# ninalu/urlearning-cpp

Measured on AMD Instinct MI355X. Metric: cBIC parent-set scores/sec + A* expansions/sec, n=25 full skeleton, higher is better.
Workload: dtype f64; 1 GPU; C3 cBIC scoring: n=25, N=10000, max-parents k=6, lambda=2.0, full n x n skeleton, 25 variables balanced over 1 GPU(s), one all-gather of the lists; config_id=c3, mode=shard, parallelism=variable shard x1, steps_in_flight=3

## Files before the change

urlearning-cpp_amd/csrc/cbic.hip:

```cpp
#include <cstdio>
#include <atomic>
#include <thread>
#include <algorithm>
#include <chrono>
#include <cmath>
#include <cstdlib>
#include <cstring>

#include "search_internal.h"
#include "host_walk.h"
#include "cbic_dev.h"

using namespace ulg;

namespace {

typedef double f64x4 __attribute__((ext_vector_type(4)));

constexpr int kGramRows = 1024;


__device__ double block_sum(double v, double *red) {
    red[threadIdx.x] = v;
    __syncthreads();
// ... 82 lines not shown


struct ScoreArgs {
    const double *gram;
    const uint32_t *binom;
    const uint8_t *cand;
    const int *meta;
    const uint64_t *tbl_off;
    const uint64_t *work;
    uint64_t total;
    float *table;
    float *hsub;
    uint64_t *queue;
    unsigned long long *qcount;
    unsigned long long *err;
    uint8_t *qkey;
    double N;
    double pen;
    int n, nv, S;
    int xcd;
    int hsub_out;
    const uint32_t *lut;
    const int32_t *lut_off;
};

__device__ __forceinline__ uint32_t xcd_block(uint32_t b, uint32_t nb, int on) {
    if (!on) return b;
    const uint32_t x = b & 7u, k = b >> 3, q = nb >> 3, r = nb & 7u;
    return x * q + (x < r ? x : r) + k;
}

__host__ __device__ inline bool cons_violates(const uint64_t *ct, int nv, int vi, uint64_t set) {
    const uint64_t b = ct[vi], e = ct[vi + 1];
    if (b == e) return false;
    const uint64_t *p = ct + nv + 1 + 2 * b;
    for (uint64_t i = 0; i < e - b; ++i)
        if ((p[2 * i] & ~set) == 0 && (p[2 * i + 1] & set) == 0) return false;
    return true;
}
template <int THREADS>
__device__ __forceinline__ const uint64_t *cons_stage(unsigned char *smem, int lds_end, const uint64_t *cons,
                                                      int cons_words) {
    if (cons_words > kConsLdsWords) return cons;
    uint64_t *sc = reinterpret_cast<uint64_t *>(smem + ((lds_end + 15) & ~15));
    for (int i = threadIdx.x; i < cons_words; i += THREADS) sc[i] = cons[i];
    return sc;
}


struct LdsLayout {
    int gram, binom, work, lutoff, toff, meta, cand, stack, bits, cmp, cmp2, total;
};
constexpr int kCmpEntryBytes = 8 + 4 + 4 + 4 + 4;
__host__ __device__ inline int align16(int x) { return (x + 15) & ~15; }
#ifndef ULG_LDS_ALIAS
#define ULG_LDS_ALIAS 1
#endif
__host__ __device__ inline LdsLayout lds_layout(int n, int nv, int S, int L, int V) {
    LdsLayout l;
    if (ULG_LDS_ALIAS && (V & 208) == 208 && bits_words(L) < 4) {
        const int W = bits_words(L);
        l.binom = 0;
        l.toff = align16(l.binom + 64 * kBinomK * 4);
        l.meta = align16(l.toff + (nv * S + 1) * 8);
        l.cmp = align16(l.meta + nv * 4 * 4);
        const int ra = l.cmp + 16;
        l.gram = ra;
        l.work = align16(l.gram + n * n * 8);
        l.lutoff = l.work + (nv + 1) * 8;
        l.cand = align16(l.lutoff + nv * 4);
        l.stack = l.bits = align16(l.cand + nv * 64);
        l.cmp2 = align16(ra + kBlock * kCmpEntryBytes);
        const int endc = l.cmp2 + 2 * W * kBlock * 8;
        l.total = l.stack > endc ? l.stack : endc;
        return l;
    }
    l.gram = 0;
    l.binom = align16(l.gram + n * n * 8);
    l.work = align16(l.binom + 64 * kBinomK * 4);
    l.lutoff = l.work + (nv + 1) * 8;
    l.toff = align16(l.lutoff + nv * 4);
    l.meta = align16(l.toff + (nv * S + 1) * 8);
    l.cand = align16(l.meta + nv * 4 * 4);
    l.stack = align16(l.cand + nv * 64);
    l.bits = l.stack;
    const int W = bits_words(L);
    l.cmp = align16(l.bits + (W >= 4 ? 3 * W * kBlock * 8 : 0));
    l.cmp2 = align16(l.cmp + ((V & 80) == 80 ? 16 + kBlock * kCmpEntryBytes : 0));
    l.total = l.cmp2 + ((V & 208) == 208 && W < 4 ? 2 * W * kBlock * 8 : 0);
    return l;
}



constexpr unsigned long long kErrWide = 1ull, kErrQueue = 2ull, kErrSlot = 4ull;
__device__ __forceinline__ uint64_t walk_segment() { return blockIdx.x % seg_count(gridDim.x); }

template <int L, int PHASE, int W>
__device__ __forceinline__ uint32_t walk_key(const uint64_t (&ow)[W]) {
    constexpr uint32_t root = PHASE == 0 ? ((1u << L) - 1u) : (((1u << L) - 1u) << 1);
    constexpr int off = PHASE == 0 ? 0 : 1;
    uint32_t key = 0;
#pragma unroll
    for (int a = 0; a < L; ++a) {
        const uint32_t t = root ^ (1u << (a + off));
        key |= (uint32_t)((ow[t >> 6] >> (t & 63u)) & 1ull) << a;
    }
    if (key == (1u << L) - 1u) {
        uint32_t sec = 0;
        int nb = 0;
#pragma unroll
        for (int a = 0; a < L; ++a)
#pragma unroll
// ... 2085 lines not shown
        if (cnt == 0) continue;
        if ((cnt + kBlock - 1) / kBlock > 0x7fffffffull)
            return set_err(k.c, ULG_ERR_UNSUPPORTED, "ulg_cbic_score: layer too large");
        const size_t wo = p.work_offset(g, L, ph);
        wide.push_back(wide_group(k, g, L, ph, k.d_wk + wo, p.group_work().data() + wo, cnt));
    }
    return wide.empty() ? ULG_OK : score_wide_groups(k, L, ph, wide, k.c->wide_pinned);
}

int launch_prologue(const ScoreCall &k) {
    ulg_ctx *c = k.c;
    const CbicPlan &p = k.p;
    const uint64_t nqc = p.zero_q ? p.nqc : 0;
    const uint64_t nz = std::max<uint64_t>((uint64_t)p.nv, std::max<uint64_t>(nqc, p.nqseg));
    const dim3 grid((unsigned)((nz + 255) / 256)), block(256);
    unsigned long long *qcount = p.zero_q ? c->d_qcount.p : nullptr, *qseg = p.zero_q ? c->d_qseg.p : nullptr;
    if (k.cons.words)
        return launch_kernel(c, call_prologue_cons_kernel, grid, block, 0, c->stream, "call_prologue", c->d_tbl_off.p,
                             p.nv, k.ls.S, c->table.p, qcount, nqc, qseg, p.nqseg, k.cons.dev, k.ls.n);
    return launch_kernel(c, call_prologue_kernel, grid, block, 0, c->stream, "call_prologue", c->d_tbl_off.p, p.nv,
                         k.ls.S, c->table.p, qcount, nqc, qseg, p.nqseg);
}

int launch_small(const ScoreCall &k, int L, int ph) {
    ulg_ctx *c = k.c;
    const CbicPlan &p = k.p;
    const int n = k.ls.n, nv = p.nv, S = k.ls.S;
    ScoreArgs ss = k.sa;
    if (L <= p.Lf) {
        if (L != 1 || ph != 0) return ULG_OK;
        ss.hsub_out = p.Lf < p.kmax;
        return launch_twin(c, k.cons, small_kernel<false>(p.Lf), small_kernel<true>(p.Lf), dim3((unsigned)nv),
                           dim3(kFusedThreads), lds_layout(n, nv, S, p.Lf, 65).total, c->stream, "score_small_fused",
                           ss, (const uint64_t *)c->d_work.p);
    }
    const size_t wo = p.work_offset(0, L, ph);
    const uint64_t cnt = p.work[wo + nv];
    if (cnt == 0) return ULG_OK;
    ss.work = c->d_work.p + wo;
    ss.total = cnt;
    ss.lut_off = p.lut_any ? c->d_lutoff.p + p.lut_offset(L, ph) : nullptr;
    ss.hsub_out = !(L == p.kmax && ph == 1);
    return launch_twin(c, k.cons, layer_kernel<false>(L, ph, p.vsmall), layer_kernel<true>(L, ph, p.vsmall),
                       dim3((unsigned)((cnt + kBlock - 1) / kBlock)), dim3(kBlock),
                       lds_layout(n, nv, S, L, p.vsmall).total, c->stream, kLayerNames[ph][L], ss);
}

int walk_bucketed(const ScoreCall &k, int g, int L, int ph, const ScoreArgs &sa, uint64_t blocks, int wk) {
    ulg_ctx *c = k.c;
    const CbicPlan &p = k.p;
    hipStream_t st = k.gst[g];
    const unsigned long long *qc = sa.qcount;
    const uint64_t nseg = seg_count(blocks);
    const int kl = L == 6 ? (wk >= 8 ? 8 : 4) : (wk >= 4 ? 4 : 2);
    uint32_t *kbase = c->d_qoffs.p + (size_t)g * kBucketMax * p.nseg_max;
    uint32_t *sidx = c->d_qsidx.p + (size_t)g * p.qcap;
    uint32_t *qaux = c->d_qaux.p + (size_t)g * p.qcap;
    const unsigned int *hdr = reinterpret_cast<const unsigned int *>(qc + nseg * kSegStride);
    prof_begin_s(c, kWalkNames[ph][L], st);
    walk_bucket_count_kernel<<<(unsigned)((nseg + kBucketSegs - 1) / kBucketSegs), 256, 0, st>>>(
        qc, (uint32_t)nseg, L, sa.qkey, qaux, kbase);
    const uint64_t items = nseg * (kSegEntries / 256);
    walk_bucket_scatter_kernel<<<(unsigned)std::min<uint64_t>(items, 2048), 256, 0, st>>>(qc, qaux, kbase,
                                                                                          (uint32_t)nseg, L, sidx);
// ... 19 lines not shown
                       sa.hsub_out ? sa.hsub : nullptr, wck ? c->d_dump.p : nullptr, k.ls.total_slots, sa.err);
    prof_end_s(c, st);
    if (wck && (rc = dump_walk_clock(c, st, sb, wck, L, ph))) return rc;
    if (wck && std::getenv("ULG_WALK_QUEUE_DUMP") &&
        (rc = dump_walk_queue(c, st, sa.queue, sa.qcount, seg_count(blocks), bits_words(L), k.ls.total_slots, wck, L,
                              ph)))
        return rc;
    return ULG_OK;
}

int launch_unrolled(const ScoreCall &k, int g, int L, int ph) {
    ulg_ctx *c = k.c;
    const CbicPlan &p = k.p;
    const uint64_t cnt = p.launch_count(g, L, ph);
    if (cnt == 0) return ULG_OK;
    const uint64_t blocks = (cnt + kBlock - 1) / kBlock;
    if (blocks > 0x7fffffffull) return set_err(c, ULG_ERR_UNSUPPORTED, "ulg_cbic_score: layer too large");
    const bool two_pass = (p.variant & 16) != 0;
    const bool bk = p.bucket && (L == 5 || L == 6);
    ScoreArgs sa = k.sa;
    sa.work = k.d_wk + p.work_offset(g, L, ph);
    sa.total = cnt;
    sa.lut_off = p.lut_any ? c->d_lutoff.p + p.lut_offset(L, ph) : nullptr;
    sa.queue = two_pass ? c->d_queue.p + (size_t)g * p.qwords : nullptr;
    sa.qcount = two_pass ? c->d_qseg.p + p.segoff[p.seg_slot(g, L, ph)] : nullptr;
    sa.qkey = bk ? c->d_qkey.p + (size_t)g * p.qcap : nullptr;
    sa.hsub_out = !(L == p.kmax && ph == 1);
    int rc;
    if ((rc = launch_twin(c, k.cons, layer_kernel<false>(L, ph, p.variant), layer_kernel<true>(L, ph, p.variant),
                          dim3((unsigned)blocks), dim3(kBlock), lds_layout(k.ls.n, p.nv, k.ls.S, L, p.variant).total,
                          k.gst[g], kLayerNames[ph][L], sa)))
        return rc;
    if (!two_pass) return ULG_OK;
    const int wk = sliced_k(L, cnt, (uint64_t)c->walk_small_sets, c->walk_k6);
    if (bk) return walk_bucketed(k, g, L, ph, sa, blocks, wk);
    if ((p.variant & 32) && sliced_fn(L, ph, wk)) return walk_sliced(k, g, L, ph, sa, blocks, wk);
    return ULG_OK;
}

int launch_layers(const ScoreCall &k, int &done_L) {
    ulg_ctx *c = k.c;
    const CbicPlan &p = k.p;
    const int G = p.G, kmax = p.kmax;
    const auto t_call = std::chrono::steady_clock::now();
    int rc;
    bool forked = false;
// ... 73 lines not shown
        (rc = ensure(c, c->gram, (size_t)(n * n))) || (rc = ensure(c, c->colstat, (size_t)(2 * n))) ||
        (rc = ensure(c, c->partials, (size_t)chunks * tiles * tiles * 256)))
        return rc;
    ULG_HIP(c, hipMemcpyAsync(c->raw.p, data, sizeof(double) * (size_t)(N * n), hipMemcpyHostToDevice, c->stream));
    prof_begin(c, "colstats");
    colstats_kernel<<<n, kBlock, 0, c->stream>>>(c->raw.p, N, c->colstat.p);
    prof_end(c);
    const int64_t tot = N * c->npad;
    prof_begin(c, "normalise");
    normalise_kernel<<<(unsigned)((tot + kBlock - 1) / kBlock), kBlock, 0, c->stream>>>(c->raw.p, N, n, c->npad,
                                                                                         c->colstat.p, c->z.p);
    prof_end(c);
    prof_begin(c, "gram_mfma_f64");
    gram_mfma_kernel<<<dim3(chunks, tiles * tiles), 64, 0, c->stream>>>(c->z.p, N, c->npad, tiles, c->partials.p);
    prof_end(c);
    prof_begin(c, "gram_reduce");
    gram_reduce_kernel<<<(n * n + kBlock - 1) / kBlock, kBlock, 0, c->stream>>>(c->partials.p, chunks, tiles, n,
                                                                               c->gram.p);
    prof_end(c);
    if ((rc = ensure(c, c->d_pen, 1))) return rc;
    penalty_kernel<<<1, 1, 0, c->stream>>>((double)N, lambda, c->d_pen.p);
    ULG_HIP(c, hipGetLastError());
    ULG_HIP(c, hipMemcpyAsync(&c->pen, c->d_pen.p, sizeof(double), hipMemcpyDeviceToHost, c->stream));
    ULG_HIP(c, hipStreamSynchronize(c->stream));
    prof_collect(c);
    c->loaded = true;
    return ULG_OK;
}

int ulg_cbic_gram(ulg_ctx *c, double *out) {
    if (!c || !out) return ULG_ERR_ARG;
    if (!c->loaded) return set_err(c, ULG_ERR_STATE, "ulg_cbic_gram: no data loaded");
    ULG_HIP(c, hipSetDevice(c->device));
    ULG_HIP(c, hipMemcpy(out, c->gram.p, sizeof(double) * (size_t)(c->n * c->n), hipMemcpyDeviceToHost));
    return ULG_OK;
}

int ulg_cbic_score_finish(ulg_ctx *c, int64_t *total_stored, int64_t *total_scored) {
    if (!c) return ULG_ERR_ARG;
    if (c->async_pending) {
        c->async_pending = false;
        ULG_HIP(c, hipSetDevice(c->device));
        ULG_HIP(c, hipStreamSynchronize(c->stream));
        prof_collect(c);
        c->total_stored = (int64_t)c->async_pinned[0];
        c->last_err_word = c->async_pinned[1];
// ... 86 lines not shown
            if (c->wide_pinned) (void)hipHostFree(c->wide_pinned);
            c->wide_pinned = nullptr;
            ULG_HIP(c, hipHostMalloc((void **)&c->wide_pinned, sizeof(unsigned long long) * 2 * (size_t)G,
                                     hipHostMallocDefault));
            c->wide_host.assign(2 * G, 0);
        }
    }
    return ensure(c, c->d_blk, (size_t)p.nb + 2);
}

void graph_key(const ulg_ctx *c, const ScoreLists &ls, const CbicPlan &p, const uint64_t *candidates,
               std::vector<uint64_t> &gkey) {
    auto ptr = [](const void *q) { return (uint64_t)(uintptr_t)q; };
    gkey.assign({(uint64_t)ls.nv, (uint64_t)ls.max_parents, (uint64_t)p.variant, (uint64_t)p.G, (uint64_t)p.Ls,
                 (uint64_t)c->score_xcd, (uint64_t)ls.n, (uint64_t)c->N, dbits(c->lambda), (uint64_t)c->prof,
                 (uint64_t)c->walk_small_sets, (uint64_t)c->walk_k6, (uint64_t)c->walk_bucket, ptr(c->d_qaux.p),
                 ptr(c->d_qsidx.p), ptr(c->d_qkey.p), ptr(c->d_qoffs.p), ptr(c->table.p), ptr(c->d_work.p),
                 ptr(c->d_workg.p), ptr(c->d_queue.p), ptr(c->d_qcount.p), ptr(c->d_qseg.p), ptr(c->d_cand.p),
                 ptr(c->d_meta.p), ptr(c->d_tbl_off.p), ptr(c->out_sets.p), ptr(c->out_scores.p),
                 ptr(c->out_offsets.p), ptr(c->d_blk.p), ptr(c->gram.p), ptr(c->d_binom.p), ptr(c->d_binom64.p),
                 ptr(c->d_hsub.p), (uint64_t)ls.total_slots, (uint64_t)c->score_small_layers, (uint64_t)c->score_fused,
                 (uint64_t)p.cons_words, ptr(p.cons_words ? c->d_cons.p : nullptr), dbits(c->pen),
                 (uint64_t)c->score_unrank_lut, ptr(p.lut_any ? c->d_lut.p : nullptr),
                 ptr(p.lut_any ? c->d_lutoff.p : nullptr)});
    for (int i = 0; i < ls.nv; ++i) gkey.push_back((uint64_t)ls.vars[i]);
    for (int i = 0; i < ls.nv; ++i) gkey.push_back(candidates[i]);
    for (const std::string &nm : c->prof_only) gkey.push_back(std::hash<std::string>{}(nm));
}

int compact(const ScoreCall &k, int done_L) {
    ulg_ctx *c = k.c;
    const ScoreLists &ls = k.ls;
    const int nv = ls.nv, S = ls.S;
    const int64_t nb = k.p.nb;
    for (int i = 0; i < nv && done_L < ls.kmax; ++i) {
        const uint64_t b = ls.toff[(size_t)i * S + done_L + 1], e = ls.toff[(size_t)i * S + S];
        if (e > b) ULG_HIP(c, hipMemsetAsync(c->table.p + b, 0xff, (size_t)(e - b) * 4, c->stream));
    }
    c->completed_layer = done_L;
    prof_begin(c, "count_stored");
    count_kernel<<<(unsigned)nb, kBlock, 0, c->stream>>>(c->table.p, ls.total_slots, c->d_blk.p);
    prof_end(c);
    prof_begin(c, "scan_stored");
    scan_kernel<<<1, 1024, 0, c->stream>>>(c->d_blk.p, nb, c->out_offsets.p + nv, k.errf());
    prof_end(c);
    const WriteArgs wa{c->table.p,      c->d_blk.p,    c->d_tbl_off.p,  c->d_meta.p,      c->d_cand.p, c->d_binom.p,
                       c->d_binom64.p,  ls.total_slots, nv,             S,                c->out_sets.p,
// ... 76 lines not shown

int cbic_score(ulg_ctx *c, const int *vars, int nv, const uint64_t *candidates, int max_parents,
               int64_t *total_stored, int64_t *total_scored, bool async) {
    if (!c) return ULG_ERR_ARG;
    if (int rc0 = finish_pending(c)) return rc0;
    if (!c->loaded) return set_err(c, ULG_ERR_STATE, "ulg_cbic_score: call ulg_cbic_load first");
    ScoreLists &ls = c->lists;
    CbicPlan &p = c->plan;
    if (ScoreLists::Status st = ls.build(c->n, vars, nv, candidates, max_parents))
        return lists_error(c, "ulg_cbic_score", st);
    ULG_HIP(c, hipSetDevice(c->device));
    CbicOptions o;
    o.score_variant = c->score_variant;
    o.score_streams = c->score_streams;
    o.score_small_layers = c->score_small_layers;
    o.score_fused = c->score_fused;
    o.walk_bucket = c->walk_bucket;
    o.wide_prune = c->wide_prune;
    o.wide_pool = c->wide_pool;
    o.time_limit_ms = c->time_limit_ms;
    const char *wck = std::getenv("ULG_WALK_CLOCK");
    o.wck = wck != nullptr;
    o.score_unrank_lut = c->score_unrank_lut;
    p.build(ls, c->cons_var, c->cons_req, c->cons_forb, o);
    LutCache staged = c->lut_cache;
    p.build_luts(ls, o.score_unrank_lut, staged);
    if (int rc = reserve_buffers(c, ls, p)) return rc;
    if (int rc = reserve_luts(c, p, staged)) return rc;

    ScoreCall k{c, ls, p, ConsTable{p.cons_words ? c->d_cons.p : nullptr, p.cons_words, p.cons_lds}, ScoreArgs{},
                p.G > 1 ? c->d_workg.p : c->d_work.p, std::vector<hipStream_t>(p.G), wck};
    k.gst[0] = c->stream;
    for (int g = 1; g < p.G; ++g) k.gst[g] = c->aux_streams[g - 1];
    ScoreArgs &sa = k.sa;
    sa.hsub_out = 1;
    sa.gram = c->gram.p;
    sa.binom = c->d_binom.p;
    sa.cand = c->d_cand.p;
    sa.meta = c->d_meta.p;
    sa.tbl_off = c->d_tbl_off.p;
    sa.table = c->table.p;
    sa.hsub = (p.variant & 64) ? c->d_hsub.p : nullptr;
    sa.err = k.errf();
    sa.N = (double)c->N;
    sa.pen = c->pen;
    sa.lut = p.lut_any ? c->d_lut.p : nullptr;
    sa.n = ls.n;
    sa.nv = ls.nv;
    sa.S = ls.S;
    sa.xcd = c->score_xcd;
    if (int rc = launch_call(k, candidates)) return rc;
// ... 147 lines not shown
```

urlearning-cpp_amd/csrc/cbic_score_layer.inc:

```
template <int L, int PHASE, int V>
__global__ void __launch_bounds__(kBlock, (score_min_waves<L, PHASE, V>()))
#if ULG_CONS
score_layer_cons_kernel(ScoreArgs a, const uint64_t *cons, int cons_words) {
#else
score_layer_kernel(ScoreArgs a) {
#endif
    extern __shared__ __attribute__((aligned(16))) unsigned char smem[];
    const LdsLayout lay = lds_layout(a.n, a.nv, a.S, L, V);
#if ULG_CONS
    const uint64_t *ct = cons_stage<kBlock>(smem, lay.total, cons, cons_words);
#endif
    double *g = reinterpret_cast<double *>(smem + lay.gram);
    uint32_t *binom = reinterpret_cast<uint32_t *>(smem + lay.binom);
    uint64_t *work = reinterpret_cast<uint64_t *>(smem + lay.work);
    uint64_t *toff = reinterpret_cast<uint64_t *>(smem + lay.toff);
    int *smeta = reinterpret_cast<int *>(smem + lay.meta);
    uint8_t *scand = reinterpret_cast<uint8_t *>(smem + lay.cand);
    constexpr bool HM = (V & 64) != 0;
    constexpr bool CMP = HM && (V & 16) != 0;
    const uint64_t gid0 = (uint64_t)xcd_block(blockIdx.x, gridDim.x, a.xcd) * kBlock + threadIdx.x;
    const WaveVar wv = wave_variable(a.work, a.lut_off, a.nv, a.total, gid0 - (threadIdx.x & 63u));
    const bool valid = gid0 < wv.total;
    const uint64_t gid = valid ? gid0 : wv.total - 1;
    bool have_um = false;
    uint32_t um = 0u;
    if (wv.vi >= 0 && wv.loff >= 0) {
        um = a.lut[(uint32_t)wv.loff + (uint32_t)(gid - wv.base)];
        have_um = true;
    }
    for (int i = threadIdx.x; i < a.n * a.n; i += kBlock) g[i] = a.gram[i];
    for (int i = threadIdx.x; i < 64 * kBinomK; i += kBlock) binom[i] = a.binom[i];
    for (int i = threadIdx.x; i <= a.nv; i += kBlock) work[i] = a.work[i];
    int32_t *slut = reinterpret_cast<int32_t *>(smem + lay.lutoff);
    if (a.lut_off)
        for (int i = threadIdx.x; i < a.nv; i += kBlock) slut[i] = a.lut_off[i];
    for (int i = threadIdx.x; i <= a.nv * a.S; i += kBlock) toff[i] = a.tbl_off[i];
    for (int i = threadIdx.x; i < a.nv * 4; i += kBlock) smeta[i] = a.meta[i];
    for (int i = threadIdx.x; i < a.nv * 16; i += kBlock)
        reinterpret_cast<uint32_t *>(scand)[i] = reinterpret_cast<const uint32_t *>(a.cand)[i];
    __syncthreads();

    if (!CMP && !valid) return;
    int vi = wv.vi;
    uint64_t r = gid - wv.base;
    if (wv.vi < 0) {
        int lo = 0, hi = a.nv;
        while (hi - lo > 1) {
            const int mid = (lo + hi) >> 1;
            if (work[mid] <= gid) lo = mid; else hi = mid;
        }
        vi = lo;
        r = gid - work[vi];
        if (a.lut_off) {
            const int32_t lo2 = slut[vi];
            if (lo2 >= 0) {
                um = a.lut[(uint32_t)lo2 + (uint32_t)r];
                have_um = true;
            }
        }
    }
    const SetHead<L> hd = set_head<L, PHASE, !CMP>(smeta, scand, binom, vi, r, have_um, um);
    const bool z = hd.z;
// ... 196 lines not shown
```

urlearning-cpp_amd/csrc/score_plan.h:

```cpp
#pragma once

#include <algorithm>
#include <cstddef>
#include <cstdint>
#include <vector>

#include "../../include/ulg.h"

#if defined(__HIPCC__)
#define ULG_HD __host__ __device__
#else
#define ULG_HD
#endif

namespace ulg {

constexpr int kMaxVars = 63;
constexpr int kMaxL = ULG_UNROLLED_PARENTS_GPU;
constexpr int kWideMax = ULG_MAX_PARENTS_GPU;

constexpr int kBlock = 256;

constexpr int kConsLdsWords = 256;

constexpr int kSegBlocks = 32;
constexpr uint64_t kSegEntries = (uint64_t)kSegBlocks * kBlock;
constexpr int kSegStride = 16;
constexpr int kBucketHdrWords = 128;
constexpr int kBucketMax = 128;
constexpr uint64_t kWideBitsWords = 1ull << 27;
constexpr int kHiMaxBits = 24;
constexpr int kSlotsPerThread = 16;
constexpr int kSlotsPerBlock = kBlock * kSlotsPerThread;

ULG_HD inline uint64_t seg_count(uint64_t blocks) { return (blocks + kSegBlocks - 1) / kSegBlocks; }
ULG_HD constexpr int bits_words(int L) { return (L + 1) <= 6 ? 1 : (1 << ((L + 1) - 6)); }

inline uint64_t binom64(int a, int b) {
    if (b < 0 || b > a) return 0;
    if (b > a - b) b = a - b;
    unsigned __int128 r = 1;
    for (int i = 1; i <= b; ++i) r = r * (unsigned)(a - b + i) / (unsigned)i;
    return r > ~0ull ? ~0ull : (uint64_t)r;
}

struct ScoreLists {
    enum Status { kOk = 0, kBadList, kNotDistinct, kTooWide };

    int n = 0, nv = 0;
    int max_parents = 0;
    int kmax = 0, S = 0;
    std::vector<int> vars;
    std::vector<uint64_t> cmask;
    std::vector<uint8_t> cand;
    std::vector<int> mv;
    std::vector<uint64_t> toff;
    uint64_t total_slots = 0;

    Status build(int n_, const int *vars_, int nv_, const uint64_t *candidates, int max_parents_) {
// ... 103 lines not shown
        for (const LutTable &t : tables)
            if (t.U == U && t.l == l) return &t;
        return nullptr;
    }
};
inline bool lut_pair(int m, bool z, int L, int ph, int &U, int &l) {
    if (ph == 0 && !z) return false;
    U = (ph == 0 || z) ? m - 1 : m;
    l = ph == 0 ? L - 1 : L;
    return l >= 0 && l <= U;
}

struct CbicOptions {
    int score_variant = 241;
    int score_streams = 3;
    int score_small_layers = 4;
    int score_fused = 3;
    int walk_bucket = 1;
    int wide_prune = 1;
    int wide_pool = 2;
    int64_t time_limit_ms = 0;
    bool wck = false;
    int64_t score_unrank_lut = kLutDefaultCap;
};

struct CbicPlan {
    int nv = 0, kmax = 0;
    std::vector<int> meta;
    size_t wstride = 0;
    std::vector<uint64_t> work;
    int variant = 0;
    int G = 1;
    std::vector<uint64_t> workg;
    uint64_t qwords = 0;
    uint64_t wqwords = 0;
    std::vector<uint64_t> segoff;
    size_t nqc = 0;
    bool bucket = false;
    uint64_t qcap = 0;
    uint64_t nseg_max = 1;
    uint64_t wave_cap = 0;
    bool zero_q = false;
    uint64_t nqseg = 0;
    uint64_t wslice = 0;
    std::vector<uint64_t> hoff;
    uint64_t htot = 0;
// ... 21 lines not shown
        if (cap <= 0 || top < kLutMinL) return;
        lutoff.assign((size_t)(kmax + 1) * 2 * nv, -1);
        for (int i = 0; i < nv; ++i)
            for (int L = kLutMinL; L <= top; ++L)
                for (int ph = 0; ph < 2; ++ph) {
                    int U, l;
                    if (!lut_pair(ls.mv[i], meta[i * 4 + 2] != 0, L, ph, U, l) || U > kLutMaxU) continue;
                    const uint64_t cnt = binom64(U, l);
                    if (cnt == 0 || cnt > (uint64_t)cap) continue;
                    const LutTable *t = cache.find(U, l);
                    if (!t) {
                        if (cache.total + cnt > kLutMaxTotal) continue;
                        cache.tables.push_back(LutTable{U, l, cache.total, cnt});
                        cache.total += cnt;
                        lut_new.push_back(cache.tables.back());
                        t = &cache.tables.back();
                    }
                    lutoff[lut_offset(L, ph) + i] = (int32_t)t->off;
                    lut_any = true;
                }
        if (!lut_any) lutoff.clear();
    }

    size_t work_offset(int g, int L, int ph) const {
        return (size_t)g * (G > 1 ? wstride : 0) + ((size_t)L * 2 + ph) * (nv + 1);
    }
    const std::vector<uint64_t> &group_work() const { return G > 1 ? workg : work; }
    uint64_t launch_count(int g, int L, int ph) const { return group_work()[work_offset(g, L, ph) + nv]; }
    size_t seg_slot(int g, int L, int ph) const { return (size_t)g * 2 * (kmax + 1) + (size_t)L * 2 + ph; }
    size_t hmeta_stride() const { return nv + (size_t)(nv + 1) * 8; }

    void build(const ScoreLists &ls, const std::vector<int> &cons_var, const std::vector<uint64_t> &cons_req,
               const std::vector<uint64_t> &cons_forb, const CbicOptions &o) {
        nv = ls.nv;
        kmax = ls.kmax;
        const std::vector<int> &mv = ls.mv;
        const int max_parents = ls.max_parents;
        meta.assign((size_t)nv * 4, 0);
        for (int i = 0; i < nv; ++i) {
            meta[i * 4 + 0] = ls.vars[i];
            meta[i * 4 + 1] = mv[i];
            meta[i * 4 + 2] = (ls.cmask[i] & 1ull) ? 1 : 0;
        }
        wstride = (size_t)(kmax + 1) * 2 * (nv + 1);
        work.assign(wstride, 0);
        for (int L = 1; L <= kmax; ++L)
// ... 145 lines not shown
```

urlearning-cpp_amd/csrc/ulg_ctx.cpp:

```cpp
#include <mutex>
#include <cstdio>
#include <cstring>

#include "disc_bdeu.h"
#include "search_internal.h"

namespace ulg {

int set_err(ulg_ctx *c, int code, const std::string &msg) {
    if (c) {
        std::lock_guard<std::mutex> lk(c->mu);
        c->err = msg;
    }
    return code;
}

const std::vector<uint32_t> &host_binom() {
    static std::vector<uint32_t> t = [] {
        std::vector<uint32_t> b(64 * kBinomK, 0);
        for (int a = 0; a < 64; ++a)
            for (int k = 0; k < kBinomK; ++k) {
                uint64_t v = binom64(a, k);
                b[a * kBinomK + k] = v > 0xFFFFFFFFull ? 0xFFFFFFFFu : (uint32_t)v;
            }
// ... 110 lines not shown

void ulg_destroy(ulg_ctx *c) {
    if (!c) return;
    (void)hipSetDevice(c->device);
    if (c->stream) (void)hipStreamSynchronize(c->stream);
    graph_reset(c);
    if (c->wide_pinned) (void)hipHostFree(c->wide_pinned);
    c->wide_pinned = nullptr;
    if (c->async_pinned) (void)hipHostFree(c->async_pinned);
    c->async_pinned = nullptr;
    for (hipEvent_t e : c->event_pool) (void)hipEventDestroy(e);
    c->event_pool.clear();
    for (hipStream_t s : c->aux_streams) (void)hipStreamDestroy(s);
    c->aux_streams.clear();
    for (hipEvent_t e : c->sync_events) (void)hipEventDestroy(e);
    c->sync_events.clear();
    release(c->raw); release(c->z); release(c->gram); release(c->partials); release(c->colstat);
    release(c->table); release(c->d_tbl_off); release(c->d_work); release(c->d_blk);
    release(c->d_cand); release(c->d_meta); release(c->d_binom); release(c->d_binom64); release(c->d_wqueue); release(c->d_wbits); release(c->d_stats); release(c->d_dump); release(c->d_queue); release(c->d_qcount); release(c->d_workg); release(c->d_vwork); release(c->d_hq); release(c->d_hqc); release(c->d_hmax); release(c->d_hoff); release(c->d_hmeta); release(c->d_scount); release(c->d_hsub); release(c->d_qseg);
    release(c->d_qaux); release(c->d_qsidx); release(c->d_qoffs); release(c->d_qkey);
    release(c->out_sets); release(c->out_scores); release(c->out_offsets);
    release(c->qbuf_in); release(c->qbuf_out);
    release(c->d_cons); release(c->d_cons_var);
    release(c->d_lut); release(c->d_lutoff); release(c->d_pen);
    release(c->d_codes); release(c->d_disc_sets); release(c->d_disc_slab); release(c->d_disc_word);
    release(c->d_disc_counts); release(c->d_disc_meta); release(c->d_disc_cand); release(c->d_disc_vm);
    release(c->d_disc_table); release(c->d_disc_blk); release(c->d_disc_best);
    release(c->d_g2_tests); release(c->d_g2_out);
    pss_release(c);
    if (c->search) {
        c->search->release_all();
        delete c->search;
        c->search = nullptr;
    }
    if (c->stream) (void)hipStreamDestroy(c->stream);
    delete c;
}

const char *ulg_last_error(const ulg_ctx *c) { return c ? c->err.c_str() : "null context"; }

int ulg_disc_set_ess(ulg_ctx *c, double ess) {
    if (!c) return ULG_ERR_ARG;
    if (!(ess >= ulg::kBdeuEssMin && ess <= ulg::kBdeuEssMax))
        return set_err(c, ULG_ERR_ARG, "ulg_disc_set_ess: ess must be finite, 1e-6 <= ess <= 1e6");
    c->disc_ess = ess;
    return ULG_OK;
}
// ... 2 lines not shown
    if (!c || !name) return ULG_ERR_ARG;
    if (std::strcmp(name, "score_streams") == 0) {
        if (value < 1 || value > 4) return set_err(c, ULG_ERR_ARG, "score_streams must be 1..4");
        c->score_streams = (int)value;
        return ULG_OK;
    }
    if (std::strcmp(name, "score_small_layers") == 0) {
        if (value < 0 || value > ULG_UNROLLED_PARENTS_GPU)
            return set_err(c, ULG_ERR_ARG, "score_small_layers must be 0..8");
        c->score_small_layers = (int)value;
        return ULG_OK;
    }
    if (std::strcmp(name, "score_fused") == 0) {
        if (value < 0 || value > 4) return set_err(c, ULG_ERR_ARG, "score_fused must be 0..4");
        c->score_fused = (int)value;
        return ULG_OK;
    }
    if (std::strcmp(name, "score_unrank_lut") == 0) {
        if (value < 0 || value > (int64_t)kLutMaxTotal)
            return set_err(c, ULG_ERR_ARG, "score_unrank_lut must be 0..2^31-1");
        c->score_unrank_lut = value;
        return ULG_OK;
    }
    if (std::strcmp(name, "score_variant") == 0) {
        if (value != 1 && value != 49 && value != 65 && value != 113 && value != 241)
            return set_err(c, ULG_ERR_ARG, "score_variant must be 1, 49, 65, 113 or 241");
        c->score_variant = (int)value;
        return ULG_OK;
    }
    if (std::strcmp(name, "time_limit_ms") == 0) {
        if (value < 0) return set_err(c, ULG_ERR_ARG, "time_limit_ms must be >= 0");
        c->time_limit_ms = value;
        return ULG_OK;
    }
    if (std::strcmp(name, "disc_dense_cells") == 0) {
        if (value < 1 || value > 32768) return set_err(c, ULG_ERR_ARG, "disc_dense_cells must be 1..32768");
        c->disc_dense_cells = value;
        return ULG_OK;
    }
    if (std::strcmp(name, "disc_prune") == 0) {
        if (value != 0 && value != 1) return set_err(c, ULG_ERR_ARG, "disc_prune must be 0 or 1");
        c->disc_prune = (int)value;
        return ULG_OK;
    }
    if (std::strcmp(name, "table_budget_kb") == 0) {
        if (value < 0) return set_err(c, ULG_ERR_ARG, "table_budget_kb must be >= 0");
// ... 81 lines not shown
        if (value < 0 || value > 2) return set_err(c, ULG_ERR_ARG, "sweep_table must be 0, 1 or 2");
        c->sweep_table = (int)value;
        return ULG_OK;
    }
    return set_err(c, ULG_ERR_ARG, std::string("unknown option: ") + name);
}

int ulg_get_info(ulg_ctx *c, const char *name, int64_t *value) {
    if (!c || !name || !value) return ULG_ERR_ARG;
    if (std::strcmp(name, "out_of_time") == 0) {
        *value = c->out_of_time;
        return ULG_OK;
    }
    if (std::strcmp(name, "highest_completed_layer") == 0) {
        *value = c->completed_layer;
        return ULG_OK;
    }
    if (std::strcmp(name, "score_error_word") == 0) {
        *value = (int64_t)c->last_err_word;
        return ULG_OK;
    }
    if (std::strcmp(name, "score_unrank_lut") == 0 || std::strcmp(name, "unrank_lut_entries") == 0) {
        *value = name[0] == 's' ? c->score_unrank_lut : (int64_t)c->lut_cache.total;
        return ULG_OK;
    }
    if (std::strcmp(name, "disc_dense_sets") == 0 || std::strcmp(name, "disc_sparse_sets") == 0) {
        *value = c->disc_path_sets[name[5] == 's' ? 1 : 0];
        return ULG_OK;
    }
    if (std::strcmp(name, "disc_pruned") == 0) {
        *value = c->disc_pruned;
        return ULG_OK;
    }
    if (std::strcmp(name, "disc_mmpc_tests") == 0 || std::strcmp(name, "disc_mmpc_skipped") == 0) {
        *value = c->disc_mmpc_stat[name[10] == 's' ? 1 : 0];
        return ULG_OK;
    }
    if (std::strcmp(name, "constraints") == 0) {
        *value = (int64_t)c->cons_var.size();
        return ULG_OK;
    }
    if (std::strcmp(name, "exact_cycles") == 0) {
        *value = c->exact_pmu[0];
        return ULG_OK;
    }
    if (std::strcmp(name, "exact_instructions") == 0) {
// ... 81 lines not shown
```

urlearning-cpp_amd/csrc/ulg_internal.h:

```cpp
#pragma once

#include <mutex>
#include <hip/hip_runtime.h>

#include <cstdint>
#include <map>
#include <string>
#include <cstring>
#include <set>
#include <vector>

#include "../../include/ulg.h"
#include "score_plan.h"

namespace ulg {

constexpr int kBinomK = kMaxL + 2;
constexpr uint32_t kAbsentBits = 0xFFFFFFFFu;

template <typename T>
struct DevBuf {
    T *p = nullptr;
    size_t cap = 0;
};

struct SearchState;
struct PssState;

struct ProfRec {
    std::string name;
    hipEvent_t start, stop;
    bool graph = false;
};

struct Mirror {
    const void *dev = nullptr;
    std::vector<unsigned char> bytes;
};

}
// ... 39 lines not shown
    int wide_lds = 1;
    int wide_pool = 2;
    uint64_t wide_host_iters = 1024;
    int wide_host_threads = 16;
    uint64_t wide_host_max = 4096;
    uint64_t wide_host_first = 0;
    int wide_host_q = 0;
    int score_xcd = 1;
    int score_graph = 1;
    hipGraph_t graph = nullptr;
    hipGraphExec_t gexec = nullptr;
    std::vector<uint64_t> gkey;
    std::vector<ulg::ProfRec> gprof;
    int sweep_xcd = 1;
    ulg::DevBuf<float> table;
    ulg::DevBuf<float> d_hsub;
    double pen = 0.0;
    ulg::DevBuf<double> d_pen;
    int64_t score_unrank_lut = ulg::kLutDefaultCap;
    ulg::LutCache lut_cache;
    ulg::DevBuf<uint32_t> d_lut;
    ulg::DevBuf<int32_t> d_lutoff;
    ulg::Mirror mir_lutoff;
    ulg::DevBuf<uint64_t> d_tbl_off, d_work, d_blk;
    ulg::DevBuf<uint8_t> d_cand;
    ulg::DevBuf<int> d_meta;
    ulg::DevBuf<uint32_t> d_binom;
    ulg::DevBuf<uint64_t> d_binom64;
    ulg::DevBuf<uint64_t> d_wqueue;
    ulg::DevBuf<uint64_t> d_wbits;
    ulg::DevBuf<unsigned long long> d_stats;
    ulg::DevBuf<uint64_t> d_dump;
    ulg::DevBuf<uint64_t> d_queue;
    ulg::DevBuf<uint32_t> d_qaux, d_qsidx, d_qoffs;
    ulg::DevBuf<uint8_t> d_qkey;
    ulg::DevBuf<unsigned long long> d_qseg;
    ulg::DevBuf<unsigned long long> d_qcount;
    ulg::DevBuf<uint64_t> d_workg;
    ulg::DevBuf<uint64_t> d_vwork;
    ulg::DevBuf<uint32_t> d_hq;
    ulg::DevBuf<unsigned int> d_hqc;
    ulg::DevBuf<uint64_t> out_sets;
    ulg::DevBuf<float> out_scores;
    ulg::DevBuf<int64_t> out_offsets;

    std::vector<int> cons_var;
// ... 135 lines not shown
```

Before: 14.77 billion parent-set scores/s.

## Stage per-launch LDS image prebuilt on host for single bulk copy into shared memory

Builds a contiguous byte image on the host for each layer launch, laid out exactly like the kernel's LDS (gram, binomial table, work offsets, lut offsets, table offsets, meta, candidates), and uploads it once. The layer kernel then fills LDS with 16-byte vector copies, issuing the first four loads early so they overlap with the work lookup, instead of running seven separate scalar staging loops. To build the image, the gram matrix is copied back to the host at load time and the LDS layout code is moved into a shared header. This adds device memory for the images and host build work, and it is on by default behind a new score_lds_image option.

```diff
diff --git a/urlearning-cpp_amd/csrc/cbic.hip b/urlearning-cpp_amd/csrc/cbic.hip
--- a/urlearning-cpp_amd/csrc/cbic.hip
+++ b/urlearning-cpp_amd/csrc/cbic.hip
@@ -128,6 +128,8 @@
     int hsub_out;
     const uint32_t *lut;
     const int32_t *lut_off;
+    const uint4 *image;
+    int image16;
 };
 
 __device__ __forceinline__ uint32_t xcd_block(uint32_t b, uint32_t nb, int on) {
@@ -151,50 +153,6 @@
     uint64_t *sc = reinterpret_cast<uint64_t *>(smem + ((lds_end + 15) & ~15));
     for (int i = threadIdx.x; i < cons_words; i += THREADS) sc[i] = cons[i];
     return sc;
-}
-
-
-struct LdsLayout {
-    int gram, binom, work, lutoff, toff, meta, cand, stack, bits, cmp, cmp2, total;
-};
-constexpr int kCmpEntryBytes = 8 + 4 + 4 + 4 + 4;
-__host__ __device__ inline int align16(int x) { return (x + 15) & ~15; }
-#ifndef ULG_LDS_ALIAS
-#define ULG_LDS_ALIAS 1
-#endif
-__host__ __device__ inline LdsLayout lds_layout(int n, int nv, int S, int L, int V) {
-    LdsLayout l;
-    if (ULG_LDS_ALIAS && (V & 208) == 208 && bits_words(L) < 4) {
-        const int W = bits_words(L);
-        l.binom = 0;
-        l.toff = align16(l.binom + 64 * kBinomK * 4);
-        l.meta = align16(l.toff + (nv * S + 1) * 8);
-        l.cmp = align16(l.meta + nv * 4 * 4);
-        const int ra = l.cmp + 16;
-        l.gram = ra;
-        l.work = align16(l.gram + n * n * 8);
-        l.lutoff = l.work + (nv + 1) * 8;
-        l.cand = align16(l.lutoff + nv * 4);
-        l.stack = l.bits = align16(l.cand + nv * 64);
-        l.cmp2 = align16(ra + kBlock * kCmpEntryBytes);
-        const int endc = l.cmp2 + 2 * W * kBlock * 8;
-        l.total = l.stack > endc ? l.stack : endc;
-        return l;
-    }
-    l.gram = 0;
-    l.binom = align16(l.gram + n * n * 8);
-    l.work = align16(l.binom + 64 * kBinomK * 4);
-    l.lutoff = l.work + (nv + 1) * 8;
-    l.toff = align16(l.lutoff + nv * 4);
-    l.meta = align16(l.toff + (nv * S + 1) * 8);
-    l.cand = align16(l.meta + nv * 4 * 4);
-    l.stack = align16(l.cand + nv * 64);
-    l.bits = l.stack;
-    const int W = bits_words(L);
-    l.cmp = align16(l.bits + (W >= 4 ? 3 * W * kBlock * 8 : 0));
-    l.cmp2 = align16(l.cmp + ((V & 80) == 80 ? 16 + kBlock * kCmpEntryBytes : 0));
-    l.total = l.cmp2 + ((V & 208) == 208 && W < 4 ? 2 * W * kBlock * 8 : 0);
-    return l;
 }
 
 
@@ -2326,6 +2284,12 @@
                          k.ls.S, c->table.p, qcount, nqc, qseg, p.nqseg);
 }
 
+void set_image(const ScoreCall &k, ScoreArgs &sa, int g, int L, int ph) {
+    const int64_t at = k.p.image_offset(g, L, ph);
+    sa.image = at < 0 ? nullptr : reinterpret_cast<const uint4 *>(k.c->d_image.p + at);
+    sa.image16 = at < 0 ? 0 : k.p.image_bytes(k.ls, L) / 16;
+}
+
 int launch_small(const ScoreCall &k, int L, int ph) {
     ulg_ctx *c = k.c;
     const CbicPlan &p = k.p;
@@ -2344,6 +2308,7 @@
     ss.work = c->d_work.p + wo;
     ss.total = cnt;
     ss.lut_off = p.lut_any ? c->d_lutoff.p + p.lut_offset(L, ph) : nullptr;
+    set_image(k, ss, 0, L, ph);
     ss.hsub_out = !(L == p.kmax && ph == 1);
     return launch_twin(c, k.cons, layer_kernel<false>(L, ph, p.vsmall), layer_kernel<true>(L, ph, p.vsmall),
                        dim3((unsigned)((cnt + kBlock - 1) / kBlock)), dim3(kBlock),
@@ -2409,6 +2374,7 @@
     sa.work = k.d_wk + p.work_offset(g, L, ph);
     sa.total = cnt;
     sa.lut_off = p.lut_any ? c->d_lutoff.p + p.lut_offset(L, ph) : nullptr;
+    set_image(k, sa, g, L, ph);
     sa.queue = two_pass ? c->d_queue.p + (size_t)g * p.qwords : nullptr;
     sa.qcount = two_pass ? c->d_qseg.p + p.segoff[p.seg_slot(g, L, ph)] : nullptr;
     sa.qkey = bk ? c->d_qkey.p + (size_t)g * p.qcap : nullptr;
@@ -2528,6 +2494,9 @@
     penalty_kernel<<<1, 1, 0, c->stream>>>((double)N, lambda, c->d_pen.p);
     ULG_HIP(c, hipGetLastError());
     ULG_HIP(c, hipMemcpyAsync(&c->pen, c->d_pen.p, sizeof(double), hipMemcpyDeviceToHost, c->stream));
+    c->h_gram.resize((size_t)n * n);
+    ULG_HIP(c, hipMemcpyAsync(c->h_gram.data(), c->gram.p, sizeof(double) * (size_t)n * n, hipMemcpyDeviceToHost,
+                              c->stream));
     ULG_HIP(c, hipStreamSynchronize(c->stream));
     prof_collect(c);
     c->loaded = true;
@@ -2660,7 +2629,8 @@
                  ptr(c->d_hsub.p), (uint64_t)ls.total_slots, (uint64_t)c->score_small_layers, (uint64_t)c->score_fused,
                  (uint64_t)p.cons_words, ptr(p.cons_words ? c->d_cons.p : nullptr), dbits(c->pen),
                  (uint64_t)c->score_unrank_lut, ptr(p.lut_any ? c->d_lut.p : nullptr),
-                 ptr(p.lut_any ? c->d_lutoff.p : nullptr)});
+                 ptr(p.lut_any ? c->d_lutoff.p : nullptr), (uint64_t)c->score_lds_image,
+                 ptr(p.image_any ? c->d_image.p : nullptr)});
     for (int i = 0; i < ls.nv; ++i) gkey.push_back((uint64_t)ls.vars[i]);
     for (int i = 0; i < ls.nv; ++i) gkey.push_back(candidates[i]);
     for (const std::string &nm : c->prof_only) gkey.push_back(std::hash<std::string>{}(nm));
@@ -2783,11 +2753,15 @@
     const char *wck = std::getenv("ULG_WALK_CLOCK");
     o.wck = wck != nullptr;
     o.score_unrank_lut = c->score_unrank_lut;
+    o.score_lds_image = c->score_lds_image;
     p.build(ls, c->cons_var, c->cons_req, c->cons_forb, o);
     LutCache staged = c->lut_cache;
     p.build_luts(ls, o.score_unrank_lut, staged);
     if (int rc = reserve_buffers(c, ls, p)) return rc;
     if (int rc = reserve_luts(c, p, staged)) return rc;
+    p.build_images(ls, c->h_gram.data(), host_binom().data(), c->score_lds_image != 0);
+    if (p.image_any)
+        if (int rc = upload(c, c->d_image, c->mir_image, p.image)) return rc;
 
     ScoreCall k{c, ls, p, ConsTable{p.cons_words ? c->d_cons.p : nullptr, p.cons_words, p.cons_lds}, ScoreArgs{},
                 p.G > 1 ? c->d_workg.p : c->d_work.p, std::vector<hipStream_t>(p.G), wck};
diff --git a/urlearning-cpp_amd/csrc/cbic_score_layer.inc b/urlearning-cpp_amd/csrc/cbic_score_layer.inc
--- a/urlearning-cpp_amd/csrc/cbic_score_layer.inc
+++ b/urlearning-cpp_amd/csrc/cbic_score_layer.inc
@@ -18,6 +18,14 @@
     uint8_t *scand = reinterpret_cast<uint8_t *>(smem + lay.cand);
     constexpr bool HM = (V & 64) != 0;
     constexpr bool CMP = HM && (V & 16) != 0;
+    const uint32_t n16 = (uint32_t)a.image16;
+    const auto piece = [&](uint32_t j) {
+        const uint32_t i = threadIdx.x + j * kBlock, at = (i < n16 ? i : n16 - 1u) << 4;
+        return (a.image && j * kBlock < n16)
+                   ? *reinterpret_cast<const uint4 *>(reinterpret_cast<const unsigned char *>(a.image) + at)
+                   : uint4{0u, 0u, 0u, 0u};
+    };
+    const uint4 im0 = piece(0), im1 = piece(1), im2 = piece(2), im3 = piece(3);
     const uint64_t gid0 = (uint64_t)xcd_block(blockIdx.x, gridDim.x, a.xcd) * kBlock + threadIdx.x;
     const WaveVar wv = wave_variable(a.work, a.lut_off, a.nv, a.total, gid0 - (threadIdx.x & 63u));
     const bool valid = gid0 < wv.total;
@@ -28,16 +36,26 @@
         um = a.lut[(uint32_t)wv.loff + (uint32_t)(gid - wv.base)];
         have_um = true;
     }
-    for (int i = threadIdx.x; i < a.n * a.n; i += kBlock) g[i] = a.gram[i];
-    for (int i = threadIdx.x; i < 64 * kBinomK; i += kBlock) binom[i] = a.binom[i];
-    for (int i = threadIdx.x; i <= a.nv; i += kBlock) work[i] = a.work[i];
     int32_t *slut = reinterpret_cast<int32_t *>(smem + lay.lutoff);
-    if (a.lut_off)
-        for (int i = threadIdx.x; i < a.nv; i += kBlock) slut[i] = a.lut_off[i];
-    for (int i = threadIdx.x; i <= a.nv * a.S; i += kBlock) toff[i] = a.tbl_off[i];
-    for (int i = threadIdx.x; i < a.nv * 4; i += kBlock) smeta[i] = a.meta[i];
-    for (int i = threadIdx.x; i < a.nv * 16; i += kBlock)
-        reinterpret_cast<uint32_t *>(scand)[i] = reinterpret_cast<const uint32_t *>(a.cand)[i];
+    if (a.image) {
+        uint4 *simg = reinterpret_cast<uint4 *>(smem);
+        const uint32_t t = threadIdx.x;
+        if (t < n16) simg[t] = im0;
+        if (t + kBlock < n16) simg[t + kBlock] = im1;
+        if (t + 2u * kBlock < n16) simg[t + 2u * kBlock] = im2;
+        if (t + 3u * kBlock < n16) simg[t + 3u * kBlock] = im3;
+        for (uint32_t i = threadIdx.x + 4u * kBlock; i < n16; i += kBlock) simg[i] = a.image[i];
+    } else {
+        for (int i = threadIdx.x; i < a.n * a.n; i += kBlock) g[i] = a.gram[i];
+        for (int i = threadIdx.x; i < 64 * kBinomK; i += kBlock) binom[i] = a.binom[i];
+        for (int i = threadIdx.x; i <= a.nv; i += kBlock) work[i] = a.work[i];
+        if (a.lut_off)
+            for (int i = threadIdx.x; i < a.nv; i += kBlock) slut[i] = a.lut_off[i];
+        for (int i = threadIdx.x; i <= a.nv * a.S; i += kBlock) toff[i] = a.tbl_off[i];
+        for (int i = threadIdx.x; i < a.nv * 4; i += kBlock) smeta[i] = a.meta[i];
+        for (int i = threadIdx.x; i < a.nv * 16; i += kBlock)
+            reinterpret_cast<uint32_t *>(scand)[i] = reinterpret_cast<const uint32_t *>(a.cand)[i];
+    }
     __syncthreads();
 
     if (!CMP && !valid) return;
diff --git a/urlearning-cpp_amd/csrc/score_plan.h b/urlearning-cpp_amd/csrc/score_plan.h
--- a/urlearning-cpp_amd/csrc/score_plan.h
+++ b/urlearning-cpp_amd/csrc/score_plan.h
@@ -3,6 +3,7 @@
 #include <algorithm>
 #include <cstddef>
 #include <cstdint>
+#include <cstring>
 #include <vector>
 
 #include "../../include/ulg.h"
@@ -35,6 +36,51 @@
 
 ULG_HD inline uint64_t seg_count(uint64_t blocks) { return (blocks + kSegBlocks - 1) / kSegBlocks; }
 ULG_HD constexpr int bits_words(int L) { return (L + 1) <= 6 ? 1 : (1 << ((L + 1) - 6)); }
+
+constexpr int kBinomK = kMaxL + 2;
+
+struct LdsLayout {
+    int gram, binom, work, lutoff, toff, meta, cand, stack, bits, cmp, cmp2, total;
+};
+constexpr int kCmpEntryBytes = 8 + 4 + 4 + 4 + 4;
+ULG_HD inline int align16(int x) { return (x + 15) & ~15; }
+#ifndef ULG_LDS_ALIAS
+#define ULG_LDS_ALIAS 1
+#endif
+ULG_HD inline LdsLayout lds_layout(int n, int nv, int S, int L, int V) {
+    LdsLayout l;
+    if (ULG_LDS_ALIAS && (V & 208) == 208 && bits_words(L) < 4) {
+        const int W = bits_words(L);
+        l.binom = 0;
+        l.toff = align16(l.binom + 64 * kBinomK * 4);
+        l.meta = align16(l.toff + (nv * S + 1) * 8);
+        l.cmp = align16(l.meta + nv * 4 * 4);
+        const int ra = l.cmp + 16;
+        l.gram = ra;
+        l.work = align16(l.gram + n * n * 8);
+        l.lutoff = l.work + (nv + 1) * 8;
+        l.cand = align16(l.lutoff + nv * 4);
+        l.stack = l.bits = align16(l.cand + nv * 64);
+        l.cmp2 = align16(ra + kBlock * kCmpEntryBytes);
+        const int endc = l.cmp2 + 2 * W * kBlock * 8;
+        l.total = l.stack > endc ? l.stack : endc;
+        return l;
+    }
+    l.gram = 0;
+    l.binom = align16(l.gram + n * n * 8);
+    l.work = align16(l.binom + 64 * kBinomK * 4);
+    l.lutoff = l.work + (nv + 1) * 8;
+    l.toff = align16(l.lutoff + nv * 4);
+    l.meta = align16(l.toff + (nv * S + 1) * 8);
+    l.cand = align16(l.meta + nv * 4 * 4);
+    l.stack = align16(l.cand + nv * 64);
+    l.bits = l.stack;
+    const int W = bits_words(L);
+    l.cmp = align16(l.bits + (W >= 4 ? 3 * W * kBlock * 8 : 0));
+    l.cmp2 = align16(l.cmp + ((V & 80) == 80 ? 16 + kBlock * kCmpEntryBytes : 0));
+    l.total = l.cmp2 + ((V & 208) == 208 && W < 4 ? 2 * W * kBlock * 8 : 0);
+    return l;
+}
 
 inline uint64_t binom64(int a, int b) {
     if (b < 0 || b > a) return 0;
@@ -184,6 +230,7 @@
     int64_t time_limit_ms = 0;
     bool wck = false;
     int64_t score_unrank_lut = kLutDefaultCap;
+    int score_lds_image = 1;
 };
 
 struct CbicPlan {
@@ -251,6 +298,45 @@
         if (!lut_any) lutoff.clear();
     }
 
+    std::vector<unsigned char> image;
+    std::vector<int64_t> imgoff;
+    bool image_any = false;
+    int64_t image_offset(int g, int L, int ph) const { return image_any ? imgoff[seg_slot(g, L, ph)] : -1; }
+    int launch_variant(int L) const { return L <= Ls ? vsmall : variant; }
+    const uint64_t *launch_work(int g, int L, int ph) const {
+        return L <= Ls ? &work[work_offset(0, L, ph)] : &group_work()[work_offset(g, L, ph)];
+    }
+    int image_bytes(const ScoreLists &ls, int L) const { return lds_layout(ls.n, nv, ls.S, L, launch_variant(L)).stack; }
+
+    void build_images(const ScoreLists &ls, const double *gram, const uint32_t *binom, bool on) {
+        image.clear();
+        imgoff.clear();
+        image_any = false;
+        const int top = std::min(kmax, kMaxL);
+        if (!on || !gram || !binom || top <= Lf) return;
+        imgoff.assign((size_t)G * 2 * (kmax + 1), -1);
+        const int n = ls.n, S = ls.S;
+        for (int L = Lf + 1; L <= top; ++L)
+            for (int ph = 0; ph < 2; ++ph)
+                for (int g = 0; g < (L <= Ls ? 1 : G); ++g) {
+                    const uint64_t *w = launch_work(g, L, ph);
+                    if (w[nv] == 0) continue;
+                    const LdsLayout lay = lds_layout(n, nv, S, L, launch_variant(L));
+                    const size_t at = image.size();
+                    image.resize(at + (size_t)lay.stack, 0);
+                    unsigned char *im = image.data() + at;
+                    std::memcpy(im + lay.gram, gram, (size_t)n * n * 8);
+                    std::memcpy(im + lay.binom, binom, (size_t)64 * kBinomK * 4);
+                    std::memcpy(im + lay.work, w, (size_t)(nv + 1) * 8);
+                    if (lut_any) std::memcpy(im + lay.lutoff, &lutoff[lut_offset(L, ph)], (size_t)nv * 4);
+                    std::memcpy(im + lay.toff, ls.toff.data(), ((size_t)nv * S + 1) * 8);
+                    std::memcpy(im + lay.meta, meta.data(), (size_t)nv * 16);
+                    std::memcpy(im + lay.cand, ls.cand.data(), (size_t)nv * 64);
+                    imgoff[seg_slot(g, L, ph)] = (int64_t)at;
+                    image_any = true;
+                }
+    }
+
     size_t work_offset(int g, int L, int ph) const {
         return (size_t)g * (G > 1 ? wstride : 0) + ((size_t)L * 2 + ph) * (nv + 1);
     }
diff --git a/urlearning-cpp_amd/csrc/ulg_ctx.cpp b/urlearning-cpp_amd/csrc/ulg_ctx.cpp
--- a/urlearning-cpp_amd/csrc/ulg_ctx.cpp
+++ b/urlearning-cpp_amd/csrc/ulg_ctx.cpp
@@ -156,7 +156,7 @@
     release(c->out_sets); release(c->out_scores); release(c->out_offsets);
     release(c->qbuf_in); release(c->qbuf_out);
     release(c->d_cons); release(c->d_cons_var);
-    release(c->d_lut); release(c->d_lutoff); release(c->d_pen);
+    release(c->d_lut); release(c->d_lutoff); release(c->d_image); release(c->d_pen);
     release(c->d_codes); release(c->d_disc_sets); release(c->d_disc_slab); release(c->d_disc_word);
     release(c->d_disc_counts); release(c->d_disc_meta); release(c->d_disc_cand); release(c->d_disc_vm);
     release(c->d_disc_table); release(c->d_disc_blk); release(c->d_disc_best);
@@ -205,6 +205,11 @@
         c->score_unrank_lut = value;
         return ULG_OK;
     }
+    if (std::strcmp(name, "score_lds_image") == 0) {
+        if (value != 0 && value != 1) return set_err(c, ULG_ERR_ARG, "score_lds_image must be 0 or 1");
+        c->score_lds_image = (int)value;
+        return ULG_OK;
+    }
     if (std::strcmp(name, "score_variant") == 0) {
         if (value != 1 && value != 49 && value != 65 && value != 113 && value != 241)
             return set_err(c, ULG_ERR_ARG, "score_variant must be 1, 49, 65, 113 or 241");
@@ -332,6 +337,10 @@
     }
     if (std::strcmp(name, "score_unrank_lut") == 0 || std::strcmp(name, "unrank_lut_entries") == 0) {
         *value = name[0] == 's' ? c->score_unrank_lut : (int64_t)c->lut_cache.total;
+        return ULG_OK;
+    }
+    if (std::strcmp(name, "score_lds_image") == 0 || std::strcmp(name, "lds_image_bytes") == 0) {
+        *value = name[0] == 's' ? c->score_lds_image : (int64_t)c->plan.image.size();
         return ULG_OK;
     }
     if (std::strcmp(name, "disc_dense_sets") == 0 || std::strcmp(name, "disc_sparse_sets") == 0) {
diff --git a/urlearning-cpp_amd/csrc/ulg_internal.h b/urlearning-cpp_amd/csrc/ulg_internal.h
--- a/urlearning-cpp_amd/csrc/ulg_internal.h
+++ b/urlearning-cpp_amd/csrc/ulg_internal.h
@@ -15,7 +15,6 @@
 
 namespace ulg {
 
-constexpr int kBinomK = kMaxL + 2;
 constexpr uint32_t kAbsentBits = 0xFFFFFFFFu;
 
 template <typename T>
@@ -101,6 +100,10 @@
     ulg::DevBuf<uint32_t> d_lut;
     ulg::DevBuf<int32_t> d_lutoff;
     ulg::Mirror mir_lutoff;
+    int score_lds_image = 1;
+    std::vector<double> h_gram;
+    ulg::DevBuf<unsigned char> d_image;
+    ulg::Mirror mir_image;
     ulg::DevBuf<uint64_t> d_tbl_off, d_work, d_blk;
     ulg::DevBuf<uint8_t> d_cand;
     ulg::DevBuf<int> d_meta;
diff --git a/urlearning-cpp_amd/host/lds_image_check.cpp b/urlearning-cpp_amd/host/lds_image_check.cpp
--- /dev/null
+++ b/urlearning-cpp_amd/host/lds_image_check.cpp
@@ -0,0 +1,128 @@
+#include <cstdio>
+#include <cstdlib>
+#include <cstring>
+#include <vector>
+
+#include "../csrc/score_plan.h"
+
+using namespace ulg;
+
+namespace {
+
+#define CHECK(cond)                                                                                  \
+    do {                                                                                             \
+        if (!(cond)) {                                                                               \
+            std::fprintf(stderr, "lds_image_check: %s:%d: %s fails\n", __FILE__, __LINE__, #cond); \
+            std::exit(1);                                                                            \
+        }                                                                                            \
+    } while (0)
+
+std::vector<uint32_t> table() {
+    std::vector<uint32_t> b(64 * kBinomK);
+    for (int a = 0; a < 64; ++a)
+        for (int k = 0; k < kBinomK; ++k) {
+            const uint64_t v = binom64(a, k);
+            b[a * kBinomK + k] = v > 0xffffffffull ? 0xffffffffu : (uint32_t)v;
+        }
+    return b;
+}
+
+void region(const unsigned char *im, std::vector<char> &covered, int at, const void *src, size_t bytes) {
+    CHECK(at >= 0 && (size_t)at + bytes <= covered.size());
+    CHECK(std::memcmp(im + at, src, bytes) == 0);
+    for (size_t i = 0; i < bytes; ++i) {
+        CHECK(!covered[at + i]);
+        covered[at + i] = 1;
+    }
+}
+
+}
+
+int main(int argc, char **argv) {
+    if (argc < 6) {
+        std::fprintf(stderr, "usage: lds_image_check VARIANT CAP MAXP N V:MASK...\n");
+        return 2;
+    }
+    const int variant = std::atoi(argv[1]);
+    const long long cap = std::atoll(argv[2]);
+    const int maxp = std::atoi(argv[3]), n = std::atoi(argv[4]);
+    std::vector<int> vars;
+    std::vector<uint64_t> masks;
+    for (int a = 5; a < argc; ++a) {
+        char *colon = nullptr;
+        vars.push_back((int)std::strtol(argv[a], &colon, 10));
+        if (!colon || *colon != ':') return 2;
+        masks.push_back(std::strtoull(colon + 1, nullptr, 16));
+    }
+    ScoreLists ls;
+    if (ls.build(n, vars.data(), (int)vars.size(), masks.data(), maxp) != ScoreLists::kOk) return 3;
+    CbicOptions o;
+    o.score_variant = variant;
+    o.score_unrank_lut = cap;
+    CbicPlan p;
+    LutCache cache;
+    p.build(ls, {}, {}, {}, o);
+    p.build_luts(ls, cap, cache);
+    std::vector<double> gram((size_t)n * n);
+    for (size_t i = 0; i < gram.size(); ++i) gram[i] = 1.0 + (double)i / 4096.0;
+    const std::vector<uint32_t> binom = table();
+
+    p.build_images(ls, gram.data(), binom.data(), false);
+    CHECK(!p.image_any && p.image.empty());
+    for (int L = 0; L <= p.kmax; ++L)
+        for (int ph = 0; ph < 2; ++ph) CHECK(p.image_offset(0, L, ph) < 0);
+
+    p.build_images(ls, gram.data(), binom.data(), true);
+    const int nv = p.nv, S = ls.S, top = std::min(p.kmax, kMaxL);
+    std::printf("PLAN kmax %d G %d Ls %d Lf %d variant %d vsmall %d lut %d bytes %zu\n", p.kmax, p.G, p.Ls, p.Lf,
+                p.variant, p.vsmall, p.lut_any ? 1 : 0, p.image.size());
+    CHECK(p.image.size() % 16 == 0);
+    int64_t next = 0;
+    int images = 0;
+    for (int L = 1; L <= p.kmax; ++L)
+        for (int ph = 0; ph < 2; ++ph)
+            for (int g = 0; g < p.G; ++g) {
+                const int64_t at = p.image_offset(g, L, ph);
+                const bool layer = L > p.Lf && L <= top && (L > p.Ls || g == 0);
+                const uint64_t cnt = !layer ? 0 : (L <= p.Ls ? p.work[p.work_offset(0, L, ph) + nv] : p.launch_count(g, L, ph));
+                if (cnt == 0) {
+                    CHECK(at < 0);
+                    continue;
+                }
+                CHECK(at == next);
+                const int V = L <= p.Ls ? p.vsmall : p.variant;
+                CHECK(V == p.launch_variant(L));
+                const LdsLayout lay = lds_layout(n, nv, S, L, V);
+                const int bytes = p.image_bytes(ls, L);
+                CHECK(bytes == lay.stack && bytes % 16 == 0 && at % 16 == 0);
+                CHECK((size_t)at + (size_t)bytes <= p.image.size());
+                next = at + bytes;
+                const bool aliased = lay.gram != 0;
+                CHECK(aliased == (ULG_LDS_ALIAS && (V & 208) == 208 && bits_words(L) < 4));
+                const unsigned char *im = p.image.data() + at;
+                std::vector<char> covered((size_t)bytes, 0);
+                const uint64_t *w = L <= p.Ls ? &p.work[p.work_offset(0, L, ph)] : &p.group_work()[p.work_offset(g, L, ph)];
+                region(im, covered, lay.gram, gram.data(), (size_t)n * n * 8);
+                region(im, covered, lay.binom, binom.data(), binom.size() * 4);
+                region(im, covered, lay.work, w, (size_t)(nv + 1) * 8);
+                if (p.lut_any) region(im, covered, lay.lutoff, &p.lutoff[p.lut_offset(L, ph)], (size_t)nv * 4);
+                region(im, covered, lay.toff, ls.toff.data(), ((size_t)nv * S + 1) * 8);
+                region(im, covered, lay.meta, p.meta.data(), (size_t)nv * 16);
+                region(im, covered, lay.cand, ls.cand.data(), (size_t)nv * 64);
+                size_t zeros = 0;
+                for (int i = 0; i < bytes; ++i)
+                    if (!covered[i]) {
+                        CHECK(im[i] == 0);
+                        ++zeros;
+                    }
+                if (aliased)
+                    for (int i = 0; i < 16; ++i) CHECK(!covered[lay.cmp + i]);
+                std::printf("IMG %d %d %d %lld %d %llu %d %zu\n", g, L, ph, (long long)at, bytes, (unsigned long long)cnt,
+                            aliased ? 1 : 0, zeros);
+                ++images;
+            }
+    CHECK((size_t)next == p.image.size());
+    CHECK(p.image_any == (images > 0));
+    std::printf("lds_image_check ok: %d images\n", images);
+    return 0;
+}
```

After: 15.77 billion parent-set scores/s, median of 6. +6.8%, better.
